# yanconglin/ICP-Flow

Measured on AMD Instinct MI355X. Metric: cluster-pair ICP registrations/sec, higher is better.
Workload: dtype f32

## Files before the change

icp_flow_amd/csrc/api.hip:

```cpp
#include <stdarg.h>
#include <stdio.h>
#include <stdlib.h>
#include <string.h>

#include "kernels.hpp"
#include "posefuse.hpp"
#include "kabsch.hpp"
#include "host.hpp"

using namespace icpflow;

namespace {

thread_local char g_err[512] = "";

}

namespace icpflow {
int report_error(int code, const char *message)
{
    snprintf(g_err, sizeof(g_err), "%s", message);
    return code;
}

// ... 154 lines not shown
        }
        Tinit = mem.take<float>(b * 16 * 4);
        M = mem.take<float>(b * 16 * 4);
        state = mem.take<IcpState>(b * sizeof(IcpState));
        ctrl = mem.take<IcpCtrl>(icp_ctrl_bytes(B));
        helpState = mem.take<float>(b * 32 * 4);
        helpOut = mem.take<double>((size_t)kHelpMaxWG * kHelpOutStride * 8);
        grid.H = grid_buckets(N);
        grid.origin = mem.take<float>(b * 4 * 4);
        grid.start = mem.take<int32_t>(b * ((size_t)grid.H + 1) * 4);
        grid.cursor = mem.take<int32_t>(b * (size_t)grid.H * 4);
        grid.pts = mem.take<float>(b * (size_t)N * 16);
        grid.sortX = mem.take<float>(b * (size_t)N * 16);
        grid.sortYsoa = mem.take<float>(b * 3 * (size_t)((N + 15) / 16 * 16) * 4 + 256);
        grid.sortXsoa = mem.take<float>(b * 3 * (size_t)((N + 15) / 16 * 16) * 4 + 256);
        zsortA = mem.take<float>(b * (size_t)N * 16);
        zsortC = mem.take<float>(b * (size_t)N * 16);
        voteKey = mem.take<float>(b * 8 * 4);
        voteWorkCap = vote_work_capacity(B, N);
        if (voteWorkCap != 0) { voteWork = mem.take<int32_t>(voteWorkCap * 4); pairOrder = mem.take<int32_t>(b * 4); }
        if (N > kChunkSortMinN) {
            const size_t cs = b * 2 * (size_t)chunk_sort_length(N) * 4;
            grid.ckey = mem.take<float>(cs);
            grid.cidx = mem.take<int>(cs);
            zckey = mem.take<float>(cs);
            zcidx = mem.take<int>(cs);
            pairBox = mem.take<float>(b * kPairBoxStride * 4);
        }
        grid.axis = mem.take<int32_t>(b * 4);
        grid.scoreList = mem.take<int>(b * 12 * 4);
        if (N <= kMaxSortN) {
            grid.occHdr = mem.take<float>(b * 2 * 8 * 4);
            grid.occBits = mem.take<uint32_t>(b * 2 * (size_t)kOccRings * kOccWords * 4);
        }
        if (shareScratch(B, N)) {
            grid.shareBest = mem.take<float>(b * 12 * kSweepShareSlots * 256 * 4);
            if (B <= 32767 && N <= 255 * 256) pairTab = mem.take<int32_t>(b * 4 * 4);
        }
        history = mem.take<float>(b * (size_t)kHistIters * kHistStride * 4);
        team.maxWG = 1024;
        team.wgPair = mem.take<int32_t>((size_t)team.maxWG * 4);
        team.wgRank = mem.take<int32_t>((size_t)team.maxWG * 4);
        team.teamSize = mem.take<int32_t>(b * 4);
        team.next = mem.take<int32_t>(b * 4);
        team.arrived = mem.take<unsigned int>(b * 4);
        team.mom = mem.take<double>((b < 256 ? b : 256) * 2 * (size_t)kMaxTeam * kTeamStride * 8);
        icpSplit = mem.take<int32_t>((b + 64) * 4);
        bytes = mem.total();
    }
};

const GridScratch *search_scratch(Workspace &w, int N, const Opts &o)
{
    int mode = o.search;
    if (o.arith == ICPFLOW_ARITH_FP32_REFERENCE) mode = 1;
    if (mode == 0) mode = (N >= 64 && N <= kMaxSortN) ? 3 : 1;
    if (mode == 3 && N > kMaxSortN) mode = 1;
    if (mode == 1) return nullptr;
    w.grid.mode = mode;
    w.grid.dirKeys = o.on(ICPFLOW_OPT_NO_DIR_KEYS) ? 1 : 0;
    return &w.grid;
}

int parse_options(const char *fn, const icpflow_options_t *opt, Opts &o)
{
    if (opt == nullptr) return 0;
// ... 1028 lines not shown
```

icp_flow_amd/csrc/kernels.hpp:

```cpp
#pragma once
#include <hip/hip_runtime.h>
#include <atomic>
#include <stddef.h>
#include <stdint.h>

#include "../../include/icpflow_hip.h"

namespace icpflow {

constexpr int ICPFLOW_STOP_REFERENCE_ = ICPFLOW_STOP_REFERENCE;
constexpr int ICPFLOW_STOP_PER_PAIR_ = ICPFLOW_STOP_PER_PAIR;

constexpr int kPartial = 8;
constexpr int kMaxIterCap = 1024;
constexpr int kCand = 6;
constexpr int kTopK = 5;
constexpr int kNmsKernel = 11;

struct IcpState {
    float R[9];
    float T[3];
    float rmse;
    int active;
    int iters;
// ... 143 lines not shown
hipError_t launch_scan_nn(const float *Qp, const float *Tp, int B, int NQ, int NT, int strideQ,
                          int strideT, const int32_t *lenQ, const int32_t *lenT, int sqrt_dist,
                          int64_t *idx, float *dist, hipStream_t s);

constexpr int kOccWords = 1024;
#ifndef ICPFLOW_OCC_RINGS
#define ICPFLOW_OCC_RINGS 3
#endif
constexpr int kOccRings = ICPFLOW_OCC_RINGS;
constexpr int kSweepShareSlots = 16;
struct GridScratch {
    int mode;
    int H;
    float *origin;
    int32_t *start;
    int32_t *cursor;
    float *pts;
    float *sortX;
    float *sortYsoa;
    float *sortXsoa;
    int32_t *axis;
    int dirKeys;
    float *ckey;
    int *cidx;
    const float *pairBox;
    const int32_t *pairTab;
    const int32_t *pairOrder;
    float *shareBest;
    int *shareCount;
    int shareCountClean;
    float *occHdr;
    uint32_t *occBits;
    int occReady;
    int *sweepTicket;
    int *scoreList;
    int presorted;
};
int grid_buckets(int N);
struct LaunchProfile;
struct IcpOpts {
    int arith = 0;
    bool teams = true;
    bool speculative = true;
    bool adaptiveWindows = true;
    bool persistent = true;
    bool helpers = true;
    IcpHelp help{};
    const float *initR = nullptr;
    const float *initT = nullptr;
    bool allowReflection = false;
    bool estimateScale = false;
    const float *initS = nullptr;
    LaunchProfile *profile = nullptr;
    bool ctrlCleared = false;
    bool *historyPending = nullptr;
    float *fp32Scratch = nullptr;
    bool teamPlanned = false;
    const uint8_t *pairActive = nullptr;
    bool teamsHalfGpu = false;
    bool sharedScans = true;
    bool twoLaunch = false;
    int32_t *splitScratch = nullptr;
};
bool icp_teams_wanted(const IcpTeam *team, const IcpOpts &opts, const GridScratch *grid, int B, int N, int maxIter,
                      int stopMode, const float *history);
int icp_team_workgroups(const IcpOpts &opts);
// ... 88 lines not shown
```

icp_flow_amd/csrc/nn.hip:

```cpp
#include "scan.hpp"
#include "sortdir.hpp"
#include "kernels.hpp"
#include "posefuse.hpp"

namespace icpflow {

enum ScanMode : int { MODE_SCORE = 0, MODE_CHECK = 1, MODE_EVAL = 2, MODE_NN = 3 };

struct ScanParams {
    const float *A;
    const float *C;
    const int32_t *lenA;
    const int32_t *lenC;
    const uint8_t *swap;
    int N;
    int NT;
    int strideQ, strideT;
    int njobs;
    int qblocks;
    const float *cand;
    int subBegin, subCount, prune;
    double *accum;
    int split;
    const float *poseA;
// ... 231 lines not shown

struct SweepParams {
    const float *Asoa;
    const float *Csoa;
    const int32_t *lenA, *lenC;
    const uint8_t *swap;
    const int32_t *axis;
    const float *cand;
    const float4 *sortX;
    const float *X, *Y;
    const float *poseA, *poseB;
    PoseSource fused;
    int rawSorted;
    const float *srcT;
    float thres;
    int N, NP16, njobs, qblocks;
    float r0;
    double *partial;
    int subBegin, subCount, prune;
    double *accum;
    float *shareBest;
    int *shareCount;
    int shareClean;
    int shareWindows;
    const int32_t *pairTab;
    const int32_t *pairOrder;
    const uint8_t *active;
    const double *initSum;
    const float *occHdr;
    const uint32_t *occBits;
    int listMode;
    int *list, *listCount;
    int boundBoth;
};

#ifdef ICPFLOW_OCC_STATS
__device__ unsigned long long g_occStats[12];
__device__ unsigned int g_occPair[1024];
#endif
constexpr int kSweepBlock = 256;
#ifndef ICPFLOW_SWEEP_SHARE_MIN_TARGETS
#define ICPFLOW_SWEEP_SHARE_MIN_TARGETS 512
#endif
constexpr int kSweepShareMinTargets = ICPFLOW_SWEEP_SHARE_MIN_TARGETS;
#ifndef ICPFLOW_SWEEP_FULLSCAN_MIN_TARGETS
#define ICPFLOW_SWEEP_FULLSCAN_MIN_TARGETS 2048
#endif
constexpr int kSweepFullScanMinTargets = ICPFLOW_SWEEP_FULLSCAN_MIN_TARGETS;
constexpr int kSweepShares = 8;
#ifndef ICPFLOW_SWEEP_FULLSCAN_QBLOCKS
#define ICPFLOW_SWEEP_FULLSCAN_QBLOCKS 2
#endif
constexpr int kSweepFullQb = ICPFLOW_SWEEP_FULLSCAN_QBLOCKS;
#ifndef ICPFLOW_SWEEP_FULLSCAN_MIN_NT
#define ICPFLOW_SWEEP_FULLSCAN_MIN_NT 512
#endif
constexpr int kSweepFullScanMinNt = ICPFLOW_SWEEP_FULLSCAN_MIN_NT;
static_assert(kSweepFullQb * kSweepShares <= kSweepShareSlots, "GridScratch.shareBest holds kSweepShareSlots records of 256 minima per job");
constexpr int kSweepStage = 4096;
enum SweepMode : int { SWEEP_SCORE = 0, SWEEP_CHECK = 1, SWEEP_EVAL = 2 };

#ifdef ICPFLOW_SWEEP_CLOCK
__device__ long long g_sweep_clk[4096 * 8];
#endif
template <int MODE, bool SHARE>
__device__ __forceinline__ void sweep_job(const SweepParams &p, const int lin)
{
#ifdef ICPFLOW_SWEEP_CLOCK
    const long long dbgW0 = wall_clock64(), dbgC0 = clock64();
    long long dbgC1 = 0, dbgC2 = 0;
    int dbgRounds = 0, dbgChunks = 0;
#endif
    __shared__ double red[(kSweepBlock / kWave) * kPartial];
    extern __shared__ __attribute__((aligned(16))) float keyLds[];
    int job = (lin / (8 * p.qblocks)) * 8 + (lin & 7);
    int qb = (lin >> 3) % p.qblocks;
    if (MODE == SWEEP_SCORE && p.prune) {
        const int padded = (p.njobs + 7) & ~7;
        qb = lin / padded;
        job = lin % padded;
        if (p.listMode == 2) {
            const int cnt = *p.listCount;
            qb = lin / cnt;
            job = p.list[lin % cnt];
        }
    }
    if (MODE == SWEEP_CHECK && p.initSum != nullptr) {
        const int pairs = p.njobs >> 1;
        const int half = ((pairs + 7) / 8) * 8 * p.qblocks;
        const int l = lin < half ? lin : lin - half;
        const int k = (l / (8 * p.qblocks)) * 8 + (l & 7);
        qb = (l >> 3) % p.qblocks;
        if (k >= pairs) return;
        job = k * 2 + (lin < half ? 1 : 0);
    }
    if (job >= p.njobs) return;
    const int listedAs = job;
    int b = (MODE == SWEEP_SCORE) ? job / p.subCount : job >> 1;
    const int sub = (MODE == SWEEP_SCORE) ? p.subBegin + job % p.subCount : (job & 1);
    if (SHARE && p.pairTab != nullptr && (MODE == SWEEP_SCORE || p.active == nullptr)) {
        const bool bw = (MODE == SWEEP_SCORE) ? (sub & 1) : (MODE == SWEEP_EVAL ? sub == 1 : false);
        const int e = p.pairTab[b * 4 + (MODE == SWEEP_EVAL ? 2 : 0) + (bw ? 1 : 0)];
        const int blocks = (p.shareCount != nullptr) ? ((e >> 8) & 255) : (e & 255);
        if (qb >= blocks) {
            const int bb = e >> 16;
            double *rec = p.partial + ((size_t)((MODE == SWEEP_SCORE) ? bb * 12 + sub : bb * 2 + sub) * p.qblocks + qb) * kPartial;
            if (threadIdx.x < kPartial) rec[threadIdx.x] = 0.0;
            if (MODE == SWEEP_SCORE && p.listMode == 1)
                for (int k = kPartial + threadIdx.x; k < p.qblocks * kPartial; k += kSweepBlock) rec[k] = 0.0;
            return;
        }
    }
    if (p.pairOrder != nullptr) b = p.pairOrder[b];
    job = (MODE == SWEEP_SCORE) ? b * 12 + sub : b * 2 + sub;
    if (MODE == SWEEP_SCORE && p.listMode == 1) {
        double *rec = p.partial + ((size_t)job * p.qblocks + 1) * kPartial;
        for (int k = threadIdx.x; k < (p.qblocks - 1) * kPartial; k += kSweepBlock) rec[k] = 0.0;
    }
    if (MODE == SWEEP_SCORE && p.prune == 1 && p.occBits != nullptr && qb > 0) {
        const double seen = __hip_atomic_load(p.accum + job, __ATOMIC_RELAXED, __HIP_MEMORY_SCOPE_AGENT);
        if (seen == __builtin_huge_val()) {
            double *rec = p.partial + ((size_t)job * p.qblocks + qb) * kPartial;
            if (threadIdx.x < kPartial) rec[threadIdx.x] = threadIdx.x == 0 ? __builtin_huge_val() : 0.0;
            return;
        }
    }
    if (MODE == SWEEP_CHECK && sub == 0 && p.initSum != nullptr) {
        const double t = p.initSum[b];
        if (t - t == 0.0 && (p.active == nullptr || p.active[b] != 0)) return;
    }
    const bool backward = (MODE == SWEEP_SCORE) ? (sub & 1) : (MODE == SWEEP_EVAL ? sub == 1 : false);
    const bool sw = p.swap != nullptr && p.swap[b] != 0;
    const int na = (sw ? p.lenC : p.lenA)[b], nc = (sw ? p.lenA : p.lenC)[b];
    const float *as = p.Asoa + (size_t)b * 3 * p.NP16, *cs = p.Csoa + (size_t)b * 3 * p.NP16;
    int naE = na, ncE = nc;
    if (MODE == SWEEP_EVAL && sw) {
        const float *t = as; as = cs; cs = t;
        naE = nc; ncE = na;
    }
    const float *qs = backward ? cs : as, *ts = backward ? as : cs, *ks = ts;
    if (MODE == SWEEP_EVAL) {
        const float *st = p.srcT + (size_t)b * 3 * p.NP16;
        if (!backward) qs = st;
        else { ts = st; ks = as; }
    }
    const int nq = backward ? ncE : naE, nt = backward ? naE : ncE;
    double *out = p.partial + ((size_t)job * p.qblocks + qb) * kPartial;
    const int lane = threadIdx.x & (kWave - 1), wave = threadIdx.x >> 6;
    __shared__ float boundSh;
    __shared__ int prunedSh;
    const bool off = MODE != SWEEP_SCORE && p.active != nullptr && p.active[b] == 0;
    const int nqb = (nq + kSweepBlock - 1) / kSweepBlock;
    const bool fullScan = SHARE && !off && p.shareCount != nullptr && nq > 0 && nqb <= kSweepFullQb && nt >= kSweepFullScanMinNt && p.qblocks >= 2 * nqb;
    const int shares = fullScan ? min(p.qblocks / nqb, kSweepShares) : 1;
    const int qi = fullScan ? qb % nqb : qb, si = fullScan ? qb / nqb : 0;
    if (fullScan && qb >= nqb && qb < shares * nqb) {
        if (threadIdx.x < kPartial) out[threadIdx.x] = 0.0;
        out = p.partial + ((size_t)job * p.qblocks + qi) * kPartial;
    } else
    if (off || qb * kSweepBlock >= nq) {
        if (threadIdx.x < kPartial) out[threadIdx.x] = 0.0;
        return;
    }
    if (MODE == SWEEP_SCORE && threadIdx.x == 0) prunedSh = 0;
    if (MODE == SWEEP_SCORE && p.prune && !fullScan) {
        __shared__ int leave;
        __shared__ double scanSum[12];
        if (wave == 0 && p.qblocks <= kWave) {
            const int q = min(lane, p.qblocks - 1);
            double v[11];
#pragma unroll
            for (int u = 0; u < 11; ++u) {
                const int sc = u == 0 ? 0 : u + 1;
                v[u] = (u == 0 || p.prune == 2) ? p.partial[((size_t)(b * 12 + sc) * p.qblocks + q) * kPartial] : 0.0;
            }
            if (p.boundBoth) {
                const double v1 = p.partial[((size_t)(b * 12 + 1) * p.qblocks + q) * kPartial];
                double t = 0.0;
                for (int qq = 0; qq < p.qblocks; ++qq) t += __shfl(v1, qq, kWave);
                if (lane == 0) scanSum[1] = t;
            }
#pragma unroll
            for (int u = 0; u < 11; ++u) {
                if (u > 0 && p.prune != 2) break;
                double t = 0.0;
                for (int qq = 0; qq < p.qblocks; ++qq) t += __shfl(v[u], qq, kWave);
                if (lane == 0) scanSum[u == 0 ? 0 : u + 1] = t;
            }
        }
        __syncthreads();
        if (threadIdx.x == 0) {
            double f0 = 0.0;
            if (p.qblocks <= kWave) f0 = scanSum[0];
            else for (int q = 0; q < p.qblocks; ++q) f0 += p.partial[((size_t)(b * 12 + 0) * p.qblocks + q) * kPartial];
            float bound = (float)f0 / (float)na;
            if (p.boundBoth) {
                double b0 = 0.0;
                if (p.qblocks <= kWave) b0 = scanSum[1];
                else for (int q = 0; q < p.qblocks; ++q) b0 += p.partial[((size_t)(b * 12 + 1) * p.qblocks + q) * kPartial];
                bound = fminf(bound, (float)b0 / (float)nc);
            }
            boundSh = bound;
            if (p.prune == 2) {
                bool othersOut = true;
                for (int k = 1; k < 6; ++k) {
                    double fk = 0.0, bk = 0.0;
                    if (p.qblocks <= kWave) { fk = scanSum[2 * k]; bk = scanSum[2 * k + 1]; }
                    else for (int q = 0; q < p.qblocks; ++q) {
                        fk += p.partial[((size_t)(b * 12 + 2 * k) * p.qblocks + q) * kPartial];
                        bk += p.partial[((size_t)(b * 12 + 2 * k + 1) * p.qblocks + q) * kPartial];
                    }
                    const float sk = fminf((float)fk / (float)na, (float)bk / (float)nc);
                    othersOut = othersOut && (sk > bound * 1.0001f);
                }
                leave = othersOut ? 1 : 0;
            } else {
                const double seen = __hip_atomic_load(p.accum + job, __ATOMIC_RELAXED, __HIP_MEMORY_SCOPE_AGENT);
                const float low = (float)(seen / (double)(float)(backward ? nc : na));
                leave = low > bound * 1.0001f ? 1 : 0;
            }
            if (leave) {
                out[0] = __builtin_huge_val();
                for (int k = 1; k < kPartial; ++k) out[k] = 0.0;
            }
        }
        __syncthreads();
        if (leave) return;
        if (p.prune == 1 && p.occBits != nullptr && sub != 1 && qb == 0 && p.listMode != 2) {
            __shared__ int occCount[kSweepBlock / kWave];
            __shared__ int occLeave;
            const float *t3 = p.cand + ((size_t)b * 6 + (sub >> 1)) * 3;
            const float ptx = t3[0], pty = t3[1], ptz = t3[2];
            const int role = backward ? 0 : 1;
            const float *hdr = p.occHdr + ((size_t)b * 2 + role) * 8;
            const uint32_t *bits = p.occBits + ((size_t)b * 2 + role) * kOccRings * kOccWords;
            const float gox = hdr[0], goy = hdr[1], goz = hdr[2], ginv = hdr[3], hlb = hdr[4];
            const int gnx = __float_as_int(hdr[5]), gny = __float_as_int(hdr[6]), gnz = __float_as_int(hdr[7]);
            int cnt = 0;
            if (gnx > 0) {
                for (int i = threadIdx.x; i < nq; i += kSweepBlock) {
                    float x = qs[i], y = qs[p.NP16 + i], z = qs[2 * p.NP16 + i];
                    if (!backward) { x += ptx; y += pty; z += ptz; }
                    else { x -= ptx; y -= pty; z -= ptz; }
                    const float ux = floorf((x - gox) * ginv), uy = floorf((y - goy) * ginv), uz = floorf((z - goz) * ginv);
                    const bool inside = ux >= 0.f && ux < (float)gnx && uy >= 0.f && uy < (float)gny && uz >= 0.f && uz < (float)gnz;
                    const bool finite = fabsf(x) < 1e30f && fabsf(y) < 1e30f && fabsf(z) < 1e30f;
                    int level = (finite && !inside) ? kOccRings : 0;
                    if (inside) {
                        const int c = ((int)ux * gny + (int)uy) * gnz + (int)uz;
#pragma unroll
                        for (int ring = 0; ring < kOccRings; ++ring)
                            level += ((bits[ring * kOccWords + (c >> 5)] >> (c & 31)) & 1u) == 0u ? 1 : 0;
                    }
                    cnt += level;
                }
            }
            cnt = wave_sum(cnt);
            if (lane == 0) occCount[wave] = cnt;
            __syncthreads();
            if (threadIdx.x == 0) {
                int tot = 0;
                for (int w = 0; w < kSweepBlock / kWave; ++w) tot += occCount[w];
                const float low = ((float)tot * hlb * 0.999f) / (float)(backward ? nc : na);
                occLeave = low > boundSh * 1.0001f ? 1 : 0;
#ifdef ICPFLOW_OCC_STATS
                atomicAdd(&g_occStats[0], 1ull); if (occLeave) atomicAdd(&g_occStats[1], 1ull);
                if (!occLeave && b < 1024) atomicAdd(&g_occPair[b], 1u);
                atomicAdd(&g_occStats[2], (unsigned long long)tot); atomicAdd(&g_occStats[3], (unsigned long long)nq);
                const float ratio = low / boundSh;
                atomicAdd(&g_occStats[4 + min(7, max(0, (int)(ratio * 4.0f)))], 1ull);
#endif
                if (occLeave) {
                    out[0] = __builtin_huge_val();
                    for (int k = 1; k < kPartial; ++k) out[k] = 0.0;
                    atomicAdd(p.accum + job, __builtin_huge_val());
                }
            }
            __syncthreads();
            if (occLeave) return;
        }
    }
    if (MODE == SWEEP_SCORE && p.listMode == 1) {
        if (threadIdx.x == 0) p.list[atomicAdd(p.listCount, 1)] = listedAs;
        return;
    }
    __shared__ float poseSh[16];
    if (MODE == SWEEP_CHECK) {
        if (sub == 1 && p.poseB == nullptr) {
            if (wave == 0) {
                const int n = pose_stop_iteration_wave(p.fused, lane);
                if (lane == 0) {
                    float M[16];
                    final_pose(p.fused, b, n, M);
#pragma unroll
                    for (int k = 0; k < 16; ++k) poseSh[k] = M[k];
                }
            }
// ... 188 lines not shown
        const long long now = wall_clock64();
        if (now > o[1]) { o[0] = dbgW0; o[1] = now; o[2] = dbgC1 - dbgC0; o[3] = dbgC2 - dbgC1; o[4] = dbgRounds; o[5] = nt; o[6] = nq; o[7] = qb; }
    }
#endif
    double v[kPartial];
#pragma unroll
    for (int k = 0; k < kPartial; ++k) v[k] = 0.0;
    if (live && nt > 0 && (!sharedWindow || wave == 0)) {
        const float d = sqrtf(best);
        v[0] = (double)d;
        if (MODE == SWEEP_EVAL) {
            v[1] = (d < p.thres) ? 1.0 : 0.0;
            if (!backward) { v[2] = qx; v[3] = qy; v[4] = qz; v[5] = ox; v[6] = oy; v[7] = oz; }
        }
    }
    constexpr int NV = (MODE == SWEEP_EVAL) ? kPartial : 1;
#pragma unroll
    for (int k = 0; k < NV; ++k) v[k] = wave_sum(v[k]);
    if (lane == 0)
        for (int k = 0; k < NV; ++k) red[wave * kPartial + k] = v[k];
    __syncthreads();
    if (threadIdx.x < kPartial) {
        double ssum = 0.0;
        if (threadIdx.x < NV)
            for (int w = 0; w < kSweepBlock / kWave; ++w) ssum += red[w * kPartial + threadIdx.x];
        if (MODE == SWEEP_SCORE && prunedSh != 0 && threadIdx.x == 0) ssum = __builtin_huge_val();
        out[threadIdx.x] = ssum;
    }
}

template <int MODE, bool SHARE = false>
__global__ __launch_bounds__(kSweepBlock) void sweep_scan_kernel(SweepParams p)
{
    sweep_job<MODE, SHARE>(p, (int)blockIdx.x);
}

template <int MODE, bool SHARE = false>
__global__ __launch_bounds__(kSweepBlock) void sweep_list_kernel(SweepParams p)
{
    const int entries = *p.listCount * p.qblocks;
    for (int e = (int)blockIdx.x; e < entries; e += (int)gridDim.x) {
        sweep_job<MODE, SHARE>(p, e);
        __syncthreads();
    }
}

__global__ void transform_soa_kernel(const float *__restrict__ soa, const int32_t *__restrict__ len,
                                     const float *__restrict__ pose, int NP16, float *__restrict__ out,
                                     const float *__restrict__ soaSwapped, const uint8_t *__restrict__ swap)
{
    const int b = blockIdx.y, k = blockIdx.x * blockDim.x + threadIdx.x;
    if (k >= NP16) return;
    const float *in = ((swap != nullptr && swap[b] != 0) ? soaSwapped : soa) + (size_t)b * 3 * NP16;
    float *o = out + (size_t)b * 3 * NP16;
    float x = kInf, y = kInf, z = kInf;
    if (k < len[b]) {
        const Affine a = affine_from_pose(pose + (size_t)b * 16);
        affine_apply(a, in[k], in[NP16 + k], in[2 * NP16 + k], x, y, z);
    }
    o[k] = x; o[NP16 + k] = y; o[2 * NP16 + k] = z;
}

#ifdef ICPFLOW_SWEEP_CLOCK
extern "C" int icpflow_debug_sweep_clk(long long *out32768)
{
    return (int)hipMemcpyFromSymbol(out32768, HIP_SYMBOL(g_sweep_clk), sizeof(long long) * 32768);
}
#endif
int sweep_qblocks(int maxRows) { return (maxRows + kSweepBlock - 1) / kSweepBlock; }

__global__ void sweep_pair_table_kernel(const int32_t *__restrict__ lenA, const int32_t *__restrict__ lenC,
                                        const uint8_t *__restrict__ swap, const int32_t *__restrict__ pairOrder, int B,
                                        int qblocks, int32_t *__restrict__ tab)
{
    const int k = blockIdx.x * blockDim.x + threadIdx.x;
    if (k >= B) return;
    const int b = pairOrder != nullptr ? pairOrder[k] : k;
    const bool sw = swap != nullptr && swap[b] != 0;
    const int na = (sw ? lenC : lenA)[b], nc = (sw ? lenA : lenC)[b];
    const int nqs[4] = {na, nc, lenA[b], lenC[b]}, nts[4] = {nc, na, lenC[b], lenA[b]};
#pragma unroll
    for (int d = 0; d < 4; ++d) {
        const int nq = nqs[d], nt = nts[d];
        const int nqb = (nq + kSweepBlock - 1) / kSweepBlock;
        const bool fullScan = nq > 0 && nqb <= kSweepFullQb && nt >= kSweepFullScanMinNt && qblocks >= 2 * nqb;
        const int shares = fullScan ? min(qblocks / nqb, kSweepShares) : 1;
        tab[k * 4 + d] = (b << 16) | (min(shares * nqb, 255) << 8) | min(nqb, 255);
    }
}

hipError_t launch_sweep_pair_table(const int32_t *lenA, const int32_t *lenC, const uint8_t *swap, const int32_t *pairOrder,
                                   int B, int N, int32_t *tab, hipStream_t s)
{
    if (B > 32767 || sweep_qblocks(N) > 255) return hipErrorInvalidValue;
    hipLaunchKernelGGL(sweep_pair_table_kernel, dim3((B + 255) / 256), dim3(256), 0, s, lenA, lenC, swap, pairOrder, B,
                       sweep_qblocks(N), tab);
    return hipGetLastError();
}

template <int MODE>
// ... 2 lines not shown
    p.NP16 = (p.N + kChunk - 1) / kChunk * kChunk;
    p.qblocks = sweep_qblocks(p.N);
    p.r0 = 0.15f;
#ifndef ICPFLOW_NO_SWEEP_SHARE
    p.shareWindows = 1;
#endif
#ifdef ICPFLOW_NO_SWEEP_SHARE
    p.shareCount = nullptr;
#endif
    if (p.N < kSweepFullScanMinTargets || p.shareBest == nullptr) p.shareCount = nullptr;
    if (p.shareCount != nullptr && !p.shareClean) {
        const hipError_t me = hipMemsetAsync(p.shareCount, 0, (size_t)(MODE == SWEEP_SCORE ? (p.njobs / p.subCount) * 12 : p.njobs) * kSweepFullQb * sizeof(int), s);
        if (me != hipSuccess) return me;
    }
    const int groups = (MODE == SWEEP_CHECK && p.initSum != nullptr) ? 2 * ((p.njobs / 2 + 7) / 8) : (p.njobs + 7) / 8;
    const size_t lds = (size_t)((p.NP16 < kSweepStage ? p.NP16 : kSweepStage) * 33 / 32 + 1) * sizeof(float);
    const int total = groups * 8 * p.qblocks;
    if (MODE == SWEEP_SCORE && p.listMode == 1) {
        const int first = groups * 8;
        if (p.shareWindows != 0 && p.N >= kSweepFullScanMinTargets && p.njobs <= 12 * 700)
            hipLaunchKernelGGL((sweep_scan_kernel<MODE, true>), dim3((unsigned)first), dim3(kSweepBlock), lds, s, p);
        else
            hipLaunchKernelGGL((sweep_scan_kernel<MODE, false>), dim3((unsigned)first), dim3(kSweepBlock), lds, s, p);
        return hipGetLastError();
    }
    if (MODE == SWEEP_SCORE && p.listMode == 2) {
        const int wgs = total < 8 * 256 ? total : 8 * 256;
        if (p.shareWindows != 0 && p.N >= kSweepFullScanMinTargets && p.njobs <= 12 * 700)
            hipLaunchKernelGGL((sweep_list_kernel<MODE, true>), dim3((unsigned)wgs), dim3(kSweepBlock), lds, s, p);
        else
            hipLaunchKernelGGL((sweep_list_kernel<MODE, false>), dim3((unsigned)wgs), dim3(kSweepBlock), lds, s, p);
        return hipGetLastError();
    }
    if (p.shareWindows != 0 && p.N >= kSweepFullScanMinTargets && p.njobs <= 12 * 700)
        hipLaunchKernelGGL((sweep_scan_kernel<MODE, true>), dim3((unsigned)total), dim3(kSweepBlock), lds, s, p);
    else
        hipLaunchKernelGGL((sweep_scan_kernel<MODE, false>), dim3((unsigned)total), dim3(kSweepBlock), lds, s, p);
    return hipGetLastError();
}

constexpr int kOccBlock = 256;
__device__ __forceinline__ uint32_t occ_shifted(const uint32_t *in, int w, int sh, bool up)
{
    const int q = sh >> 5, r = sh & 31;
    if (up) {
        const int a = w - q;
        const uint32_t lo = a >= 0 ? in[a] : 0u, lo1 = a - 1 >= 0 ? in[a - 1] : 0u;
        return r == 0 ? lo : ((lo << r) | (lo1 >> (32 - r)));
    }
    const int a = w + q;
    const uint32_t hi = a < kOccWords ? in[a] : 0u, hi1 = a + 1 < kOccWords ? in[a + 1] : 0u;
    return r == 0 ? hi : ((hi >> r) | (hi1 << (32 - r)));
}

__global__ __launch_bounds__(kOccBlock) void occ_build_kernel(const float *__restrict__ Xsoa, const float *__restrict__ Ysoa,
                                                            int NP16, float *__restrict__ hdrOut, uint32_t *__restrict__ bitsOut)
{
    __shared__ uint32_t bitsA[kOccWords], bitsB[kOccWords];
    __shared__ float red[6 * (kOccBlock / kWave)];
    __shared__ float hd[8];
    const int b = blockIdx.x, which = blockIdx.y, tid = threadIdx.x, lane = tid & (kWave - 1), wave = tid >> 6;
    const float *px = (which == 0 ? Xsoa : Ysoa) + (size_t)b * 3 * NP16, *py = px + NP16, *pz = py + NP16;
    for (int k = tid; k < kOccWords; k += kOccBlock) bitsA[k] = 0u;
    float mn[3] = {kInf, kInf, kInf}, mx[3] = {-kInf, -kInf, -kInf};
    for (int i = tid; i < NP16; i += kOccBlock) {
        const float x = px[i], y = py[i], z = pz[i];
        if (fabsf(x) < 1e30f && fabsf(y) < 1e30f && fabsf(z) < 1e30f) {
            mn[0] = fminf(mn[0], x); mn[1] = fminf(mn[1], y); mn[2] = fminf(mn[2], z);
            mx[0] = fmaxf(mx[0], x); mx[1] = fmaxf(mx[1], y); mx[2] = fmaxf(mx[2], z);
        }
// ... 67 lines not shown
    }
    if (tid < 8) hdrOut[((size_t)b * 2 + which) * 8 + tid] = hd[tid];
}

hipError_t launch_occupancy(const GridScratch *grid, int B, int N, hipStream_t s)
{
    if (grid->occHdr == nullptr || grid->occBits == nullptr || grid->sortXsoa == nullptr || grid->sortYsoa == nullptr) return hipSuccess;
    const int NP16 = (N + kChunk - 1) / kChunk * kChunk;
    hipLaunchKernelGGL(occ_build_kernel, dim3(B, 2), dim3(kOccBlock), 0, s, grid->sortXsoa, grid->sortYsoa, NP16, grid->occHdr, grid->occBits);
    return hipGetLastError();
}

hipError_t launch_sweep_score(const GridScratch *grid, const int32_t *lenA, const int32_t *lenC, const uint8_t *swap,
                              int B, int N, const float *cand, double *partial, hipStream_t s)
{
    SweepParams p{};
    p.Asoa = grid->sortXsoa; p.Csoa = grid->sortYsoa; p.lenA = lenA; p.lenC = lenC; p.swap = swap;
    p.axis = grid->axis; p.cand = cand; p.N = N; p.njobs = B * 12; p.partial = partial;
    p.subBegin = 0; p.subCount = 12;
    p.shareBest = grid->shareBest; p.shareCount = grid->shareCount; p.shareClean = grid->shareCountClean; p.pairOrder = grid->pairOrder; p.pairTab = grid->pairTab;
    return launch_sweep<SWEEP_SCORE>(p, s);
}

hipError_t launch_sweep_score_pruned(const GridScratch *grid, const int32_t *lenA, const int32_t *lenC,
                                     const uint8_t *swap, int B, int N, const float *cand, double *partial,
                                     double *accum, hipStream_t s)
{
    SweepParams p{};
    p.Asoa = grid->sortXsoa; p.Csoa = grid->sortYsoa; p.lenA = lenA; p.lenC = lenC; p.swap = swap;
    p.axis = grid->axis; p.cand = cand; p.N = N; p.partial = partial; p.accum = accum;
    if (grid->occReady) { p.occHdr = grid->occHdr; p.occBits = grid->occBits; }
    p.shareBest = grid->shareBest; p.shareCount = grid->shareCount; p.shareClean = grid->shareCountClean; p.pairOrder = grid->pairOrder; p.pairTab = grid->pairTab;
    if (grid->occReady) {
        p.njobs = B * 2; p.subBegin = 0; p.subCount = 2; p.prune = 0;
        hipError_t e2 = launch_sweep<SWEEP_SCORE>(p, s);
        if (e2 != hipSuccess) return e2;
        p.njobs = B * 10; p.subBegin = 2; p.subCount = 10; p.prune = 1; p.boundBoth = 1;
#ifndef ICPFLOW_SCORE_LIST_MIN_JOBS
#define ICPFLOW_SCORE_LIST_MIN_JOBS 65536
#endif
        if (grid->sweepTicket != nullptr && grid->scoreList != nullptr &&
            (long long)B * 10 * sweep_qblocks(N) >= ICPFLOW_SCORE_LIST_MIN_JOBS) {
            p.list = grid->scoreList; p.listCount = grid->sweepTicket;
            p.listMode = 1;
            const hipError_t e3 = launch_sweep<SWEEP_SCORE>(p, s);
            if (e3 != hipSuccess) return e3;
            p.listMode = 2;
        }
        return launch_sweep<SWEEP_SCORE>(p, s);
    }
    p.njobs = B; p.subBegin = 0; p.subCount = 1; p.prune = 0;
    hipError_t e = launch_sweep<SWEEP_SCORE>(p, s);
    if (e != hipSuccess) return e;
    p.njobs = B * 11; p.subBegin = 1; p.subCount = 11; p.prune = 1;
    return launch_sweep<SWEEP_SCORE>(p, s);
}

hipError_t launch_sweep_eval(const GridScratch *grid, const int32_t *len1, const int32_t *len2, int B, int N,
                             const float *pose, float thres, float *srcT, double *partial, hipStream_t s,
                             const uint8_t *swap, const uint8_t *active)
{
    SweepParams p{};
    p.active = active;
    p.Asoa = grid->sortXsoa; p.Csoa = grid->sortYsoa; p.lenA = len1; p.lenC = len2; p.axis = grid->axis;
    p.swap = swap;
    p.poseA = pose; p.thres = thres; p.srcT = srcT; p.N = N; p.njobs = B * 2; p.partial = partial;
    p.shareBest = grid->shareBest; p.shareCount = grid->shareCount; p.shareClean = grid->shareCountClean; p.pairOrder = grid->pairOrder; p.pairTab = grid->pairTab;
    const int NP16 = (N + kChunk - 1) / kChunk * kChunk;
    hipLaunchKernelGGL(transform_soa_kernel, dim3((NP16 + 255) / 256, B), dim3(256), 0, s, grid->sortXsoa, len1, pose,
                       NP16, srcT, grid->sortYsoa, swap);
    return launch_sweep<SWEEP_EVAL>(p, s);
}

hipError_t launch_sweep_check(const GridScratch *grid, const float *X, const float *Y, const int32_t *lenA,
                              const int32_t *lenC, const uint8_t *swap, int B, int N, const float *poseInit,
// ... 109 lines not shown
```

Before: 403,800.

## Precompute occupancy ring totals and schedule pruned score scans per pair

The occupancy ring-level counts used for the lower-bound prune now run as extra blocks inside the first (candidate 0) sweep launch and are stored per pair and candidate. A new pair-oriented kernel then decides, per pair, which of the ten remaining scans survive the bound and assigns blocks only to surviving scans, with a slot layout that can run whole scans in one block for small query counts. The goal is to avoid launching blocks that would only compute the occupancy count and exit, and to cut wasted blocks. It reuses the scoreList buffer to hold the totals and adds a dependency on the first launch having written them.

```diff
diff --git a/icp_flow_amd/csrc/api.hip b/icp_flow_amd/csrc/api.hip
--- a/icp_flow_amd/csrc/api.hip
+++ b/icp_flow_amd/csrc/api.hip
@@ -210,6 +210,7 @@
         if (N <= kMaxSortN) {
             grid.occHdr = mem.take<float>(b * 2 * 8 * 4);
             grid.occBits = mem.take<uint32_t>(b * 2 * (size_t)kOccRings * kOccWords * 4);
+            grid.occTot = grid.scoreList;
         }
         if (shareScratch(B, N)) {
             grid.shareBest = mem.take<float>(b * 12 * kSweepShareSlots * 256 * 4);
diff --git a/icp_flow_amd/csrc/kernels.hpp b/icp_flow_amd/csrc/kernels.hpp
--- a/icp_flow_amd/csrc/kernels.hpp
+++ b/icp_flow_amd/csrc/kernels.hpp
@@ -199,6 +199,7 @@
     float *occHdr;
     uint32_t *occBits;
     int occReady;
+    int32_t *occTot;
     int *sweepTicket;
     int *scoreList;
     int presorted;
diff --git a/icp_flow_amd/csrc/nn.hip b/icp_flow_amd/csrc/nn.hip
--- a/icp_flow_amd/csrc/nn.hip
+++ b/icp_flow_amd/csrc/nn.hip
@@ -287,6 +287,8 @@
     int listMode;
     int *list, *listCount;
     int boundBoth;
+    int32_t *occTot;
+    int totBase, pairSlots;
 };
 
 #ifdef ICPFLOW_OCC_STATS
@@ -316,11 +318,102 @@
 enum SweepMode : int { SWEEP_SCORE = 0, SWEEP_CHECK = 1, SWEEP_EVAL = 2 };
 
 #ifdef ICPFLOW_SWEEP_CLOCK
+__device__ long long g_sweep_blk[131072 * 2];
+__device__ __forceinline__ void sweep_blk_clock(const SweepParams &p, const long long w0)
+{
+    const int at = (p.prune == 1 ? 0 : 65536) + (int)blockIdx.x;
+    if (threadIdx.x == 0 && blockIdx.x < 65536u) { g_sweep_blk[2 * at] = w0; g_sweep_blk[2 * at + 1] = wall_clock64(); }
+}
 __device__ long long g_sweep_clk[4096 * 8];
 #endif
+__device__ __forceinline__ int sweep_ring_levels(const SweepParams &p, const int b, const int sub, const bool backward, const float *qs,
+                                                 const int nq)
+{
+    const float *t3 = p.cand + ((size_t)b * 6 + (sub >> 1)) * 3;
+    const float ptx = t3[0], pty = t3[1], ptz = t3[2];
+    const int role = backward ? 0 : 1;
+    const float *hdr = p.occHdr + ((size_t)b * 2 + role) * 8;
+    const uint32_t *bits = p.occBits + ((size_t)b * 2 + role) * kOccRings * kOccWords;
+    const float gox = hdr[0], goy = hdr[1], goz = hdr[2], ginv = hdr[3];
+    const int gnx = __float_as_int(hdr[5]), gny = __float_as_int(hdr[6]), gnz = __float_as_int(hdr[7]);
+    int cnt = 0;
+    if (gnx > 0) {
+        for (int i = threadIdx.x; i < nq; i += kSweepBlock) {
+            float x = qs[i], y = qs[p.NP16 + i], z = qs[2 * p.NP16 + i];
+            if (!backward) { x += ptx; y += pty; z += ptz; }
+            else { x -= ptx; y -= pty; z -= ptz; }
+            const float ux = floorf((x - gox) * ginv), uy = floorf((y - goy) * ginv), uz = floorf((z - goz) * ginv);
+            const bool inside = ux >= 0.f && ux < (float)gnx && uy >= 0.f && uy < (float)gny && uz >= 0.f && uz < (float)gnz;
+            const bool finite = fabsf(x) < 1e30f && fabsf(y) < 1e30f && fabsf(z) < 1e30f;
+            int level = (finite && !inside) ? kOccRings : 0;
+            if (inside) {
+                const int c = ((int)ux * gny + (int)uy) * gnz + (int)uz;
+#pragma unroll
+                for (int ring = 0; ring < kOccRings; ++ring)
+                    level += ((bits[ring * kOccWords + (c >> 5)] >> (c & 31)) & 1u) == 0u ? 1 : 0;
+            }
+            cnt += level;
+        }
+    }
+    return cnt;
+}
+
+__device__ __forceinline__ bool sweep_prebound_ends(const int tot, const float hlb, const int n, const float bound, float *lowOut = nullptr)
+{
+    const float low = ((float)tot * hlb * 0.999f) / (float)n;
+    if (lowOut != nullptr) *lowOut = low;
+    return low > bound * 1.0001f;
+}
+
+__device__ __forceinline__ float sweep_cand0_bound(const SweepParams &p, const int b, const int na, const int nc, const bool both,
+                                                   const int lane)
+{
+    const double *fw = p.partial + (size_t)(b * 12 + 0) * p.qblocks * kPartial, *bw = p.partial + (size_t)(b * 12 + 1) * p.qblocks * kPartial;
+    double f0 = 0.0, b0 = 0.0;
+    if (p.qblocks <= kWave) {
+        const int q = min(lane, p.qblocks - 1);
+        const double v0 = fw[(size_t)q * kPartial], v1 = both ? bw[(size_t)q * kPartial] : 0.0;
+        for (int qq = 0; qq < p.qblocks; ++qq) { f0 += __shfl(v0, qq, kWave); b0 += __shfl(v1, qq, kWave); }
+    } else {
+        for (int q = 0; q < p.qblocks; ++q) { f0 += fw[(size_t)q * kPartial]; if (both) b0 += bw[(size_t)q * kPartial]; }
+    }
+    float bound = (float)f0 / (float)na;
+    if (both) bound = fminf(bound, (float)b0 / (float)nc);
+    return bound;
+}
+
+struct SweepDirect {
+    int job, qb;
+    float bound;
+};
+
+__device__ __forceinline__ void sweep_tot_job(const SweepParams &p, const int lin)
+{
+    __shared__ int totCount[kSweepBlock / kWave];
+    const int k = lin / 10, sub = 2 + lin % 10;
+    const int b = p.pairOrder != nullptr ? p.pairOrder[k] : k;
+    const bool backward = (sub & 1) != 0;
+    const bool sw = p.swap != nullptr && p.swap[b] != 0;
+    const int na = (sw ? p.lenC : p.lenA)[b], nc = (sw ? p.lenA : p.lenC)[b];
+    const float *qs = (backward ? p.Csoa : p.Asoa) + (size_t)b * 3 * p.NP16;
+    int cnt = sweep_ring_levels(p, b, sub, backward, qs, backward ? nc : na);
+    cnt = wave_sum(cnt);
+    if ((threadIdx.x & (kWave - 1)) == 0) totCount[threadIdx.x >> 6] = cnt;
+    __syncthreads();
+    if (threadIdx.x == 0) {
+        int tot = 0;
+        for (int w = 0; w < kSweepBlock / kWave; ++w) tot += totCount[w];
+        p.occTot[b * 12 + sub] = tot;
+#ifdef ICPFLOW_OCC_STATS
+        atomicAdd(&g_occStats[2], (unsigned long long)tot); atomicAdd(&g_occStats[3], (unsigned long long)(backward ? nc : na));
+#endif
+    }
+}
+
 template <int MODE, bool SHARE>
-__device__ __forceinline__ void sweep_job(const SweepParams &p, const int lin)
-{
+__device__ __forceinline__ void sweep_job(const SweepParams &p, const int lin, const SweepDirect d = SweepDirect{-1, 0, 0.f})
+{
+    const bool direct = d.job >= 0;
 #ifdef ICPFLOW_SWEEP_CLOCK
     const long long dbgW0 = wall_clock64(), dbgC0 = clock64();
     long long dbgC1 = 0, dbgC2 = 0;
@@ -339,6 +432,7 @@
             qb = lin / cnt;
             job = p.list[lin % cnt];
         }
+        if (direct) { qb = d.qb; job = d.job; }
     }
     if (MODE == SWEEP_CHECK && p.initSum != nullptr) {
         const int pairs = p.njobs >> 1;
@@ -372,7 +466,7 @@
         double *rec = p.partial + ((size_t)job * p.qblocks + 1) * kPartial;
         for (int k = threadIdx.x; k < (p.qblocks - 1) * kPartial; k += kSweepBlock) rec[k] = 0.0;
     }
-    if (MODE == SWEEP_SCORE && p.prune == 1 && p.occBits != nullptr && qb > 0) {
+    if (MODE == SWEEP_SCORE && p.prune == 1 && p.occBits != nullptr && qb > 0 && !direct) {
         const double seen = __hip_atomic_load(p.accum + job, __ATOMIC_RELAXED, __HIP_MEMORY_SCOPE_AGENT);
         if (seen == __builtin_huge_val()) {
             double *rec = p.partial + ((size_t)job * p.qblocks + qb) * kPartial;
@@ -421,41 +515,26 @@
     if (MODE == SWEEP_SCORE && p.prune && !fullScan) {
         __shared__ int leave;
         __shared__ double scanSum[12];
-        if (wave == 0 && p.qblocks <= kWave) {
-            const int q = min(lane, p.qblocks - 1);
-            double v[11];
-#pragma unroll
-            for (int u = 0; u < 11; ++u) {
-                const int sc = u == 0 ? 0 : u + 1;
-                v[u] = (u == 0 || p.prune == 2) ? p.partial[((size_t)(b * 12 + sc) * p.qblocks + q) * kPartial] : 0.0;
-            }
-            if (p.boundBoth) {
-                const double v1 = p.partial[((size_t)(b * 12 + 1) * p.qblocks + q) * kPartial];
-                double t = 0.0;
-                for (int qq = 0; qq < p.qblocks; ++qq) t += __shfl(v1, qq, kWave);
-                if (lane == 0) scanSum[1] = t;
-            }
-#pragma unroll
-            for (int u = 0; u < 11; ++u) {
-                if (u > 0 && p.prune != 2) break;
-                double t = 0.0;
-                for (int qq = 0; qq < p.qblocks; ++qq) t += __shfl(v[u], qq, kWave);
-                if (lane == 0) scanSum[u == 0 ? 0 : u + 1] = t;
+        if (wave == 0 && !direct) {
+            const float bd = sweep_cand0_bound(p, b, na, nc, p.boundBoth != 0, lane);
+            if (lane == 0) boundSh = bd;
+            if (p.prune == 2 && p.qblocks <= kWave) {
+                const int q = min(lane, p.qblocks - 1);
+                double v[10];
+#pragma unroll
+                for (int u = 0; u < 10; ++u) v[u] = p.partial[((size_t)(b * 12 + 2 + u) * p.qblocks + q) * kPartial];
+#pragma unroll
+                for (int u = 0; u < 10; ++u) {
+                    double t = 0.0;
+                    for (int qq = 0; qq < p.qblocks; ++qq) t += __shfl(v[u], qq, kWave);
+                    if (lane == 0) scanSum[2 + u] = t;
+                }
             }
         }
         __syncthreads();
         if (threadIdx.x == 0) {
-            double f0 = 0.0;
-            if (p.qblocks <= kWave) f0 = scanSum[0];
-            else for (int q = 0; q < p.qblocks; ++q) f0 += p.partial[((size_t)(b * 12 + 0) * p.qblocks + q) * kPartial];
-            float bound = (float)f0 / (float)na;
-            if (p.boundBoth) {
-                double b0 = 0.0;
-                if (p.qblocks <= kWave) b0 = scanSum[1];
-                else for (int q = 0; q < p.qblocks; ++q) b0 += p.partial[((size_t)(b * 12 + 1) * p.qblocks + q) * kPartial];
-                bound = fminf(bound, (float)b0 / (float)nc);
-            }
-            boundSh = bound;
+            if (direct) boundSh = d.bound;
+            const float bound = boundSh;
             if (p.prune == 2) {
                 bool othersOut = true;
                 for (int k = 1; k < 6; ++k) {
@@ -481,43 +560,20 @@
         }
         __syncthreads();
         if (leave) return;
-        if (p.prune == 1 && p.occBits != nullptr && sub != 1 && qb == 0 && p.listMode != 2) {
+        if (p.prune == 1 && p.occBits != nullptr && sub != 1 && qb == 0 && p.listMode != 2 && !direct) {
             __shared__ int occCount[kSweepBlock / kWave];
             __shared__ int occLeave;
-            const float *t3 = p.cand + ((size_t)b * 6 + (sub >> 1)) * 3;
-            const float ptx = t3[0], pty = t3[1], ptz = t3[2];
-            const int role = backward ? 0 : 1;
-            const float *hdr = p.occHdr + ((size_t)b * 2 + role) * 8;
-            const uint32_t *bits = p.occBits + ((size_t)b * 2 + role) * kOccRings * kOccWords;
-            const float gox = hdr[0], goy = hdr[1], goz = hdr[2], ginv = hdr[3], hlb = hdr[4];
-            const int gnx = __float_as_int(hdr[5]), gny = __float_as_int(hdr[6]), gnz = __float_as_int(hdr[7]);
-            int cnt = 0;
-            if (gnx > 0) {
-                for (int i = threadIdx.x; i < nq; i += kSweepBlock) {
-                    float x = qs[i], y = qs[p.NP16 + i], z = qs[2 * p.NP16 + i];
-                    if (!backward) { x += ptx; y += pty; z += ptz; }
-                    else { x -= ptx; y -= pty; z -= ptz; }
-                    const float ux = floorf((x - gox) * ginv), uy = floorf((y - goy) * ginv), uz = floorf((z - goz) * ginv);
-                    const bool inside = ux >= 0.f && ux < (float)gnx && uy >= 0.f && uy < (float)gny && uz >= 0.f && uz < (float)gnz;
-                    const bool finite = fabsf(x) < 1e30f && fabsf(y) < 1e30f && fabsf(z) < 1e30f;
-                    int level = (finite && !inside) ? kOccRings : 0;
-                    if (inside) {
-                        const int c = ((int)ux * gny + (int)uy) * gnz + (int)uz;
-#pragma unroll
-                        for (int ring = 0; ring < kOccRings; ++ring)
-                            level += ((bits[ring * kOccWords + (c >> 5)] >> (c & 31)) & 1u) == 0u ? 1 : 0;
-                    }
-                    cnt += level;
-                }
-            }
+            const float hlb = p.occHdr[((size_t)b * 2 + (backward ? 0 : 1)) * 8 + 4];
+            int cnt = sweep_ring_levels(p, b, sub, backward, qs, nq);
             cnt = wave_sum(cnt);
             if (lane == 0) occCount[wave] = cnt;
             __syncthreads();
             if (threadIdx.x == 0) {
                 int tot = 0;
                 for (int w = 0; w < kSweepBlock / kWave; ++w) tot += occCount[w];
-                const float low = ((float)tot * hlb * 0.999f) / (float)(backward ? nc : na);
-                occLeave = low > boundSh * 1.0001f ? 1 : 0;
+                float low;
+                occLeave = sweep_prebound_ends(tot, hlb, backward ? nc : na, boundSh, &low) ? 1 : 0;
+                (void)low;
 #ifdef ICPFLOW_OCC_STATS
                 atomicAdd(&g_occStats[0], 1ull); if (occLeave) atomicAdd(&g_occStats[1], 1ull);
                 if (!occLeave && b < 1024) atomicAdd(&g_occPair[b], 1u);
@@ -772,7 +828,101 @@
 template <int MODE, bool SHARE = false>
 __global__ __launch_bounds__(kSweepBlock) void sweep_scan_kernel(SweepParams p)
 {
+#ifdef ICPFLOW_SWEEP_CLOCK
+    const long long dbgBlk0 = wall_clock64();
+#endif
+    if (MODE == SWEEP_SCORE && p.totBase > 0 && (int)blockIdx.x >= p.totBase) {
+        sweep_tot_job(p, (int)blockIdx.x - p.totBase);
+#ifdef ICPFLOW_SWEEP_CLOCK
+        sweep_blk_clock(p, dbgBlk0);
+#endif
+        return;
+    }
     sweep_job<MODE, SHARE>(p, (int)blockIdx.x);
+#ifdef ICPFLOW_SWEEP_CLOCK
+    if (MODE == SWEEP_SCORE) sweep_blk_clock(p, dbgBlk0);
+#endif
+}
+
+#ifndef ICPFLOW_SCORE_PAIR_SLOTS
+#define ICPFLOW_SCORE_PAIR_SLOTS 4
+#endif
+constexpr int kSweepPairSlots = ICPFLOW_SCORE_PAIR_SLOTS;
+static_assert(kSweepPairSlots >= 0 && kSweepPairSlots <= 10, "a pair has ten scans beside candidate 0's");
+template <bool SHARE>
+__global__ __launch_bounds__(kSweepBlock) void sweep_pair_kernel(SweepParams p)
+{
+    __shared__ float pairBound;
+    __shared__ unsigned pairGoesOn;
+#ifdef ICPFLOW_SWEEP_CLOCK
+    const long long dbgBlk0 = wall_clock64();
+#endif
+    const int lin = (int)blockIdx.x;
+    const int pairs = p.njobs / p.subCount, pairBlocks = pairs * p.qblocks;
+    const bool whole = lin >= p.pairSlots * pairBlocks;
+    const int slot = whole ? p.pairSlots + (lin - p.pairSlots * pairBlocks) / pairs : lin / pairBlocks;
+    const int k = whole ? (lin - p.pairSlots * pairBlocks) % pairs : (lin % pairBlocks) / p.qblocks;
+    const int qb = whole ? 0 : (lin % pairBlocks) % p.qblocks;
+    const int b = p.pairOrder != nullptr ? p.pairOrder[k] : k;
+    const bool sw = p.swap != nullptr && p.swap[b] != 0;
+    const int na = (sw ? p.lenC : p.lenA)[b], nc = (sw ? p.lenA : p.lenC)[b];
+    const bool sharing = SHARE && p.shareCount != nullptr;
+    bool beyond = qb > 0 && !sharing && qb * kSweepBlock >= max(na, nc);
+    if (qb > 0 && SHARE && p.pairTab != nullptr) {
+        const int e0 = p.pairTab[k * 4 + 0], e1 = p.pairTab[k * 4 + 1];
+        const int sh = sharing ? 8 : 0;
+        beyond = qb >= max((e0 >> sh) & 255, (e1 >> sh) & 255);
+    }
+    if (beyond) {
+        if (slot == 0 && threadIdx.x < 10 * kPartial)
+            p.partial[((size_t)(b * 12 + 2 + threadIdx.x / kPartial) * p.qblocks + qb) * kPartial + threadIdx.x % kPartial] = 0.0;
+#ifdef ICPFLOW_SWEEP_CLOCK
+        sweep_blk_clock(p, dbgBlk0);
+#endif
+        return;
+    }
+    if (threadIdx.x < kWave) {
+        const int lane = threadIdx.x;
+        const float bound = sweep_cand0_bound(p, b, na, nc, true, lane);
+        bool goesOn = false;
+        if (lane < 10) {
+            const int sub = 2 + lane;
+            const bool backward = (sub & 1) != 0;
+            const int nq = backward ? nc : na, nt = backward ? na : nc;
+            const int nqb = (nq + kSweepBlock - 1) / kSweepBlock;
+            const bool fullScan = sharing && nq > 0 && nqb <= kSweepFullQb && nt >= kSweepFullScanMinNt && p.qblocks >= 2 * nqb;
+            const float hlb = p.occHdr[((size_t)b * 2 + (backward ? 0 : 1)) * 8 + 4];
+            const int tot = p.occTot[b * 12 + sub];
+            goesOn = nq <= 0 || fullScan || !sweep_prebound_ends(tot, hlb, nq, bound);
+        }
+        const unsigned mask = (unsigned)(__ballot(goesOn) & 0x3ffull);
+        if (lane == 0) { pairBound = bound; pairGoesOn = mask; }
+#ifdef ICPFLOW_OCC_STATS
+        if (lane == 0 && qb == 0 && slot == 0) {
+            atomicAdd(&g_occStats[0], 10ull); atomicAdd(&g_occStats[1], (unsigned long long)(10 - __popc(mask)));
+            if (b < 1024) atomicAdd(&g_occPair[b], (unsigned)__popc(mask));
+        }
+#endif
+    }
+    __syncthreads();
+    const unsigned goesOn = pairGoesOn;
+    const float bound = pairBound;
+    if (slot == 0 && threadIdx.x < 10 * kPartial && ((goesOn >> (threadIdx.x / kPartial)) & 1u) == 0u)
+        p.partial[((size_t)(b * 12 + 2 + threadIdx.x / kPartial) * p.qblocks + qb) * kPartial + threadIdx.x % kPartial] =
+            threadIdx.x % kPartial == 0 ? __builtin_huge_val() : 0.0;
+    unsigned rest = goesOn;
+    for (int nth = 0; nth < slot && rest != 0u; ++nth) rest &= rest - 1u;
+    if (rest != 0u) {
+        const int job = k * 10 + (__ffs(rest) - 1);
+        if (!whole) sweep_job<SWEEP_SCORE, SHARE>(p, 0, SweepDirect{job, qb, bound});
+        else for (int q = 0; q < p.qblocks; ++q) {
+            sweep_job<SWEEP_SCORE, SHARE>(p, 0, SweepDirect{job, q, bound});
+            __syncthreads();
+        }
+    }
+#ifdef ICPFLOW_SWEEP_CLOCK
+    sweep_blk_clock(p, dbgBlk0);
+#endif
 }
 
 template <int MODE, bool SHARE = false>
@@ -806,6 +956,11 @@
 {
     return (int)hipMemcpyFromSymbol(out32768, HIP_SYMBOL(g_sweep_clk), sizeof(long long) * 32768);
 }
+extern "C" int icpflow_debug_sweep_blk(long long *out262144)
+{
+    return (int)hipMemcpyFromSymbol(out262144, HIP_SYMBOL(g_sweep_blk), sizeof(long long) * 262144);
+}
+extern "C" int icpflow_debug_sweep_layout(void) { return kSweepPairSlots; }
 #endif
 int sweep_qblocks(int maxRows) { return (maxRows + kSweepBlock - 1) / kSweepBlock; }
 
@@ -874,10 +1029,23 @@
             hipLaunchKernelGGL((sweep_list_kernel<MODE, false>), dim3((unsigned)wgs), dim3(kSweepBlock), lds, s, p);
         return hipGetLastError();
     }
+    if (MODE == SWEEP_SCORE && p.pairSlots > 0) {
+        const unsigned blocks = (unsigned)((p.njobs / p.subCount) * (p.qblocks * p.pairSlots + 10 - p.pairSlots));
+        if (p.shareWindows != 0 && p.N >= kSweepFullScanMinTargets && p.njobs <= 12 * 700)
+            hipLaunchKernelGGL((sweep_pair_kernel<true>), dim3(blocks), dim3(kSweepBlock), lds, s, p);
+        else
+            hipLaunchKernelGGL((sweep_pair_kernel<false>), dim3(blocks), dim3(kSweepBlock), lds, s, p);
+        return hipGetLastError();
+    }
+    unsigned blocks = (unsigned)total;
+    if (MODE == SWEEP_SCORE && p.totBase != 0) {
+        p.totBase = total;
+        blocks += (unsigned)((p.njobs / p.subCount) * 10);
+    }
     if (p.shareWindows != 0 && p.N >= kSweepFullScanMinTargets && p.njobs <= 12 * 700)
-        hipLaunchKernelGGL((sweep_scan_kernel<MODE, true>), dim3((unsigned)total), dim3(kSweepBlock), lds, s, p);
+        hipLaunchKernelGGL((sweep_scan_kernel<MODE, true>), dim3(blocks), dim3(kSweepBlock), lds, s, p);
     else
-        hipLaunchKernelGGL((sweep_scan_kernel<MODE, false>), dim3((unsigned)total), dim3(kSweepBlock), lds, s, p);
+        hipLaunchKernelGGL((sweep_scan_kernel<MODE, false>), dim3(blocks), dim3(kSweepBlock), lds, s, p);
     return hipGetLastError();
 }
 
@@ -1011,15 +1179,29 @@
     if (grid->occReady) { p.occHdr = grid->occHdr; p.occBits = grid->occBits; }
     p.shareBest = grid->shareBest; p.shareCount = grid->shareCount; p.shareClean = grid->shareCountClean; p.pairOrder = grid->pairOrder; p.pairTab = grid->pairTab;
     if (grid->occReady) {
+#ifndef ICPFLOW_SCORE_LIST_MIN_JOBS
+#define ICPFLOW_SCORE_LIST_MIN_JOBS 65536
+#endif
+        const bool listed = grid->sweepTicket != nullptr && grid->scoreList != nullptr &&
+                            (long long)B * 10 * sweep_qblocks(N) >= ICPFLOW_SCORE_LIST_MIN_JOBS;
+#ifndef ICPFLOW_SCORE_PAIR_MAX_BLOCKS
+#define ICPFLOW_SCORE_PAIR_MAX_BLOCKS 1024
+#endif
+#ifndef ICPFLOW_SCORE_PAIR_WHOLE_MAX_QBLOCKS
+#define ICPFLOW_SCORE_PAIR_WHOLE_MAX_QBLOCKS 4
+#endif
+        const bool byPair = kSweepPairSlots > 0 && !listed && grid->occTot != nullptr && (long long)B * sweep_qblocks(N) <= ICPFLOW_SCORE_PAIR_MAX_BLOCKS;
         p.njobs = B * 2; p.subBegin = 0; p.subCount = 2; p.prune = 0;
+        if (byPair) { p.occTot = grid->occTot; p.totBase = 1; }
         hipError_t e2 = launch_sweep<SWEEP_SCORE>(p, s);
         if (e2 != hipSuccess) return e2;
+        p.totBase = 0;
         p.njobs = B * 10; p.subBegin = 2; p.subCount = 10; p.prune = 1; p.boundBoth = 1;
-#ifndef ICPFLOW_SCORE_LIST_MIN_JOBS
-#define ICPFLOW_SCORE_LIST_MIN_JOBS 65536
-#endif
-        if (grid->sweepTicket != nullptr && grid->scoreList != nullptr &&
-            (long long)B * 10 * sweep_qblocks(N) >= ICPFLOW_SCORE_LIST_MIN_JOBS) {
+        if (byPair) {
+            p.pairSlots = sweep_qblocks(N) <= ICPFLOW_SCORE_PAIR_WHOLE_MAX_QBLOCKS ? kSweepPairSlots : 10;
+            return launch_sweep<SWEEP_SCORE>(p, s);
+        }
+        if (listed) {
             p.list = grid->scoreList; p.listCount = grid->sweepTicket;
             p.listMode = 1;
             const hipError_t e3 = launch_sweep<SWEEP_SCORE>(p, s);
```

Result: faster. 411,000, median of 6 (+1.8%).
